# i2nico/MDAnalysis-MPI

Hardware: AMD Instinct MI355X
Metric: atom-frames/sec (RMSF) + achieved HBM GB/s fraction (higher is better)
Workload: dtype f64

## Files before the change

include/rmsf_hip.h:

```cpp
#ifndef RMSF_HIP_H
#define RMSF_HIP_H

#include <stddef.h>
#include <stdint.h>

#ifdef __cplusplus
extern "C" {
#endif

#define RMSF_ABI_VERSION 1

#define RMSF_OK 0
#define RMSF_EINVAL (-1)
#define RMSF_EHIP (-2)
#define RMSF_ENOMEM (-3)
#define RMSF_EEMPTY (-4)

#define RMSF_MODE_WELFORD 0
#define RMSF_MODE_SUM 1

#define RMSF_XFORM_DOUBLES 16
#define RMSF_MAX_SPLIT_FRAMES 4096
#define RMSF_REFINFO_DOUBLES 2064

// ... 15 lines not shown
int rmsf_reference_setup(const float *d_frame, const double *d_avg,
                         int64_t n_sel, const int32_t *d_sel,
                         const double *d_masses, double *d_ref,
                         double *d_refinfo, void *stream);

int rmsf_reference_setup_mean(const double *d_sum, double n_frames,
                              int64_t n_sel, const double *d_masses,
                              double *d_avg, double *d_ref, double *d_refinfo,
                              void *stream);

size_t rmsf_superpose_workspace_bytes(int64_t n_sel, int64_t n_frames);
int rmsf_superpose(const float *d_xyz, int64_t frame_stride, int64_t n_frames,
                   int64_t n_sel, const int32_t *d_sel,
                   const double *d_masses, const double *d_ref,
                   const double *d_refinfo, double *d_xform, void *d_work,
                   size_t work_bytes, void *stream);

int rmsf_superpose_compact(const float *d_xyz, int64_t frame_stride,
                           int64_t n_frames, int64_t n_sel, const int32_t *d_sel,
                           const double *d_masses, const double *d_ref,
                           const double *d_refinfo, double *d_xform,
                           void *d_work, size_t work_bytes, float *d_dense_out,
                           int64_t dense_stride, void *stream);

int rmsf_superpose_planes(const float *d_xyz, int64_t frame_stride,
                          int64_t plane_stride, int64_t n_frames,
                          int64_t n_sel, const int32_t *d_sel,
                          const double *d_masses, const double *d_ref,
                          const double *d_refinfo, double *d_xform,
                          void *d_work, size_t work_bytes, void *stream);

int rmsf_accumulate_splits(int64_t n_sel, int64_t n_frames, int aligned);
int rmsf_accumulate(const float *d_xyz, int64_t frame_stride, int64_t n_frames,
                    int64_t n_sel, const int32_t *d_sel,
                    const double *d_xform, const double *d_refinfo, int mode,
                    int n_splits, double *d_out0, double *d_out1,
                    void *stream);

int64_t rmsf_split_count(int64_t n_frames, int n_splits, int s);

size_t rmsf_accumulate_balanced_workspace_bytes(int64_t n_sel, int64_t n_frames,
                                                int n_groups);
int rmsf_accumulate_balanced(const float *d_xyz, int64_t frame_stride,
                             int64_t n_frames, int64_t n_sel,
                             const int32_t *d_sel, const double *d_xform,
                             const double *d_refinfo, int mode, int n_groups,
// ... 350 lines not shown
```

mdanalysis-mpi_amd/csrc/rmsf_device.h:

```cpp
#pragma once
#include <hip/hip_runtime.h>

#include <cmath>

__device__ __forceinline__ void apply_xform(float &x, float &y, float &z, const double *__restrict__ t,
                                            double rc0, double rc1, double rc2) {
  const float p0 = (float)((double)x - t[9]);
  const float p1 = (float)((double)y - t[10]);
  const float p2 = (float)((double)z - t[11]);
  const double d0 = p0, d1 = p1, d2 = p2;
  const float r0 = (float)__builtin_fma(d2, t[6], __builtin_fma(d1, t[3], d0 * t[0]));
  const float r1 = (float)__builtin_fma(d2, t[7], __builtin_fma(d1, t[4], d0 * t[1]));
  const float r2 = (float)__builtin_fma(d2, t[8], __builtin_fma(d1, t[5], d0 * t[2]));
  x = (float)((double)r0 + rc0);
  y = (float)((double)r1 + rc1);
  z = (float)((double)r2 + rc2);
}

__host__ __device__ inline void qcp_solve(const double *A, double E0, double len, double *rot,
                                          double *rmsd) {
  const double Sxx = A[0], Sxy = A[1], Sxz = A[2];
  const double Syx = A[3], Syy = A[4], Syz = A[5];
  const double Szx = A[6], Szy = A[7], Szz = A[8];

// ... 53 lines not shown
  const double evecprec = 1e-6;
  if (qsqr < evecprec) {
    q1 = a12 * a3344_4334 - a13 * a3244_4234 + a14 * a3243_4233;
    q2 = -a11 * a3344_4334 + a13 * a3144_4134 - a14 * a3143_4133;
    q3 = a11 * a3244_4234 - a12 * a3144_4134 + a14 * a3142_4132;
    q4 = -a11 * a3243_4233 + a12 * a3143_4133 - a13 * a3142_4132;
    qsqr = q1 * q1 + q2 * q2 + q3 * q3 + q4 * q4;
    if (qsqr < evecprec) {
      const double a1324_1423 = a13 * a24 - a14 * a23, a1224_1422 = a12 * a24 - a14 * a22;
      const double a1223_1322 = a12 * a23 - a13 * a22, a1124_1421 = a11 * a24 - a14 * a21;
      const double a1123_1321 = a11 * a23 - a13 * a21, a1122_1221 = a11 * a22 - a12 * a21;
      q1 = a42 * a1324_1423 - a43 * a1224_1422 + a44 * a1223_1322;
      q2 = -a41 * a1324_1423 + a43 * a1124_1421 - a44 * a1123_1321;
      q3 = a41 * a1224_1422 - a42 * a1124_1421 + a44 * a1122_1221;
      q4 = -a41 * a1223_1322 + a42 * a1123_1321 - a43 * a1122_1221;
      qsqr = q1 * q1 + q2 * q2 + q3 * q3 + q4 * q4;
      if (qsqr < evecprec) {
        q1 = a32 * a1324_1423 - a33 * a1224_1422 + a34 * a1223_1322;
        q2 = -a31 * a1324_1423 + a33 * a1124_1421 - a34 * a1123_1321;
        q3 = a31 * a1224_1422 - a32 * a1124_1421 + a34 * a1122_1221;
        q4 = -a31 * a1223_1322 + a32 * a1123_1321 - a33 * a1122_1221;
        qsqr = q1 * q1 + q2 * q2 + q3 * q3 + q4 * q4;
        if (qsqr < evecprec) {
          rot[0] = rot[4] = rot[8] = 1.0;
          rot[1] = rot[2] = rot[3] = rot[5] = rot[6] = rot[7] = 0.0;
          return;
        }
      }
    }
  }
  const double normq = sqrt(qsqr);
  q1 /= normq;
  q2 /= normq;
  q3 /= normq;
  q4 /= normq;
  const double a2 = q1 * q1, x2 = q2 * q2, y2 = q3 * q3, z2 = q4 * q4;
  const double xy = q2 * q3, az = q1 * q4, zx = q4 * q2, ay = q1 * q3, yz = q3 * q4, ax = q1 * q2;
  rot[0] = a2 + x2 - y2 - z2;
  rot[1] = 2 * (xy + az);
  rot[2] = 2 * (zx - ay);
  rot[3] = 2 * (xy - az);
  rot[4] = a2 - x2 + y2 - z2;
  rot[5] = 2 * (yz + ax);
  rot[6] = 2 * (zx + ay);
  rot[7] = 2 * (yz - ax);
  rot[8] = a2 - x2 - y2 + z2;
}
```

mdanalysis-mpi_amd/csrc/rmsf_kernels.hip:

```cpp
#include <hip/hip_runtime.h>

#include <algorithm>
#include <cmath>
#include <cstdint>
#include <cstring>
#include <mutex>
#include <string>
#include <type_traits>
#include <unordered_map>
#include <vector>

#include "rmsf_hip.h"
#include "rmsf_device.h"

#define RMSF_EXPORT __attribute__((visibility("default")))
#ifndef RMSF_SHIFTED_SUMS
#define RMSF_SHIFTED_SUMS 1
#endif

namespace {

thread_local std::string g_err;

int fail(int code, const std::string &msg) {
// ... 2814 lines not shown
    return fail(RMSF_EINVAL, "rmsf_welford_sequential: workspace too small");
  hipStream_t s = S(stream);
  SeqCoef *coef = static_cast<SeqCoef *>(d_work);
  hipLaunchKernelGGL(k_seq_coef, dim3(grid1(n_frames)), dim3(kBlock), 0, s, k0, n_frames, coef);
  if (int rc = after_launch("k_seq_coef")) return rc;
  const int64_t n_coord = 3 * n_sel;
  if (d_sel && n_sel >= kSeqAtomsMinSel) {
    hipLaunchKernelGGL((k_welford_seq_atoms<kSeqAtomsU>), dim3(grid1(n_sel)), dim3(kBlock), 0, s, d_xyz, fstride,
                       n_frames, n_sel, d_sel, k0, coef, d_mean, d_sumsquares);
    return after_launch("k_welford_seq_atoms");
  }
  if (d_sel)
    hipLaunchKernelGGL((k_welford_seq<kSeqU, true>), dim3(grid1(n_coord)), dim3(kBlock), 0, s, d_xyz, fstride,
                       n_frames, n_coord, d_sel, k0, coef, d_mean, d_sumsquares);
  else
    hipLaunchKernelGGL((k_welford_seq<kSeqU, false>), dim3(grid1(n_coord)), dim3(kBlock), 0, s, d_xyz, fstride,
                       n_frames, n_coord, nullptr, k0, coef, d_mean, d_sumsquares);
  return after_launch("k_welford_seq");
}

}

namespace {
bool ref_seq_args_ok(const float *d_frame, const double *d_avg, double avg_divisor, int64_t n_sel,
                     const int32_t *d_sel, const double *d_ref, const double *d_refinfo) {
  return (d_frame == nullptr) != (d_avg == nullptr) && n_sel >= 1 && d_ref && d_refinfo &&
         !(d_avg && !(avg_divisor > 0.0)) && !(d_avg && d_sel);
}
template <int PART>
void ref_seq_launch(const float *d_frame, const double *d_avg, double div, int64_t n_sel, const int32_t *d_sel,
                    const double *d_masses, double mass_total, double *d_avg_out, double *d_ref, double *d_refinfo,
                    hipStream_t s) {
  const bool g = d_sel != nullptr, m = d_masses != nullptr;
#define SEQREF(F, G, M)                                                                                          \
  hipLaunchKernelGGL((k_ref_seq<F, G, M, PART>), dim3(1), dim3(kBlock), 0, s, d_frame, d_avg, div, n_sel, d_sel, \
                     d_masses, mass_total, d_avg_out, d_ref, d_refinfo)
  if (d_frame) {
    if (g && m) SEQREF(true, true, true);
    else if (g) SEQREF(true, true, false);
    else if (m) SEQREF(true, false, true);
    else SEQREF(true, false, false);
  } else {
    if (m) SEQREF(false, false, true);
    else SEQREF(false, false, false);
  }
#undef SEQREF
// ... 303 lines not shown
```

mdanalysis-mpi_amd/rmsf_amd/_lib.py:

```python
from __future__ import annotations

import ctypes
import os
from ctypes import POINTER, c_char_p, c_double, c_int, c_int32, c_int64, c_size_t, c_uint64, c_void_p

_HERE = os.path.dirname(os.path.abspath(__file__))
LIB_PATH = os.path.normpath(os.path.join(_HERE, "..", "lib", "librmsf_hip.so"))

RMSF_OK = 0
RMSF_EINVAL = -1
RMSF_EHIP = -2
RMSF_ENOMEM = -3
RMSF_EEMPTY = -4
RMSF_MODE_WELFORD = 0
RMSF_MODE_SUM = 1
RMSF_XFORM_DOUBLES = 16
RMSF_MAX_SPLIT_FRAMES = 4096
RMSF_REFINFO_DOUBLES = 2064
ABI_VERSION = 1


class RmsfError(RuntimeError):

    def __init__(self, code: int, func: str, msg: str):
        super().__init__(f"{func} failed with status {code}: {msg}")
        self.code = code


class RmsfEmptyError(RmsfError, ZeroDivisionError):
    """No frames to reduce.  Subclasses ZeroDivisionError because RMSF.py:39
    raises exactly that when two empty partials are merged."""


P = c_void_p
SIGNATURES = {
    "rmsf_abi_version": (c_int, []),
    "rmsf_last_error": (c_char_p, []),
    "rmsf_device_count": (c_int, [POINTER(c_int)]),
    "rmsf_set_device": (c_int, [c_int]),
    "rmsf_malloc": (c_int, [POINTER(c_void_p), c_size_t]),
    "rmsf_free": (c_int, [P]),
    "rmsf_memcpy_h2d": (c_int, [P, P, c_size_t, P]),
    "rmsf_memcpy_d2h": (c_int, [P, P, c_size_t, P]),
    "rmsf_memcpy2d_d2d": (c_int, [P, c_size_t, P, c_size_t, c_size_t, c_size_t, P]),
    "rmsf_stream_synchronize": (c_int, [P]),
    "rmsf_block_range": (c_int, [c_int64, c_int, c_int, POINTER(c_int64), POINTER(c_int64)]),
    "rmsf_reference_setup": (c_int, [P, P, c_int64, P, P, P, P, P]),
    "rmsf_reference_setup_mean": (c_int, [P, c_double, c_int64, P, P, P, P, P]),
    "rmsf_fold_balanced_finalize": (c_int, [P, c_int64, c_int64, P, P, c_int64, P, P]),
    "rmsf_superpose_workspace_bytes": (c_size_t, [c_int64, c_int64]),
    "rmsf_superpose": (c_int, [P, c_int64, c_int64, c_int64, P, P, P, P, P, P, c_size_t, P]),
    "rmsf_superpose_planes": (c_int, [P, c_int64, c_int64, c_int64, c_int64, P, P, P, P, P, P, c_size_t, P]),
    "rmsf_superpose_compact": (c_int, [P, c_int64, c_int64, c_int64, P, P, P, P, P, P, c_size_t, P, c_int64, P]),
    "rmsf_accumulate_splits": (c_int, [c_int64, c_int64, c_int]),
    "rmsf_accumulate": (c_int, [P, c_int64, c_int64, c_int64, P, P, P, c_int, c_int, P, P, P]),
    "rmsf_split_count": (c_int64, [c_int64, c_int, c_int]),
    "rmsf_accumulate_balanced_workspace_bytes": (c_size_t, [c_int64, c_int64, c_int]),
    "rmsf_accumulate_balanced": (c_int, [P, c_int64, c_int64, c_int64, P, P, P, c_int, c_int, P, c_size_t, P]),
    "rmsf_fold_balanced": (c_int, [P, c_int64, c_int, c_int64, P, P, P]),
    "rmsf_accumulate_balanced_planes": (c_int, [P, c_int64, c_int64, c_int64, c_int64, P, P, P, c_int, c_int, P,
                                                c_size_t, P]),
    "rmsf_chan_merge": (c_int, [P, P, P, c_int, c_int64, P, P, P]),
    "rmsf_chan_reduce_steps": (c_int, [c_int, c_int, P, P, c_int]),
    "rmsf_chan_reduce": (c_int, [P, P, P, c_int, c_int64, c_int, P, P, P]),
    "rmsf_chan_merge_pair": (c_int, [P, P, c_int64, P, P, c_int64, c_int64, P]),
    "rmsf_sum_splits": (c_int, [P, c_int, c_int64, P, P]),
    "rmsf_divide": (c_int, [P, c_double, c_int64, P, P]),
    "rmsf_chan_weight": (c_int, [P, c_double, c_int64, P, P]),
    "rmsf_chan_deviation": (c_int, [P, P, P, c_double, c_int64, P, P]),
    "rmsf_finalize": (c_int, [P, c_int64, c_int64, P, P]),
    "rmsf_reference_setup_sequential": (c_int, [P, P, c_double, c_int64, P, P, c_double, P, P, P, P]),
    "rmsf_superpose_sequential": (c_int, [P, c_int64, c_int64, c_int64, P, P, c_double, P, P, P, P]),
    "rmsf_reference_centre_sequential": (c_int, [P, P, c_double, c_int64, P, P, c_double, P, P, P, P]),
    "rmsf_reference_sums_sequential": (c_int, [c_int64, c_double, P, P, P]),
    "rmsf_frame_com_sequential": (c_int, [P, c_int64, c_int64, c_int64, P, P, c_double, P, P]),
    "rmsf_inner_product_sequential": (c_int, [P, c_int64, c_int64, c_int64, P, P, P, P]),
# ... 171 lines not shown
```

mdanalysis-mpi_amd/rmsf_amd/engine.py:

```python
from __future__ import annotations

import ctypes

import numpy as np
import torch

from . import _lib
from ._lib import RMSF_MODE_SUM, RMSF_MODE_WELFORD, RMSF_REFINFO_DOUBLES, RMSF_XFORM_DOUBLES, call

F64 = torch.float64
F32 = torch.float32


def _ptr(t: torch.Tensor | None) -> int | None:
    return None if t is None else t.data_ptr()


class Engine:

    def __init__(self, device: torch.device | int | str | None = None):
        self.lib = _lib.load()
        if not torch.cuda.is_available():
            raise RuntimeError("rmsf_amd needs a HIP device (MI355X); none is visible -- no CPU fallback exists")
        if device is None:
# ... 40 lines not shown
        info = self.empty(RMSF_REFINFO_DOUBLES)
        call("rmsf_reference_setup_mean", total.data_ptr(), float(n_frames), n_sel, _ptr(masses), avg.data_ptr(),
             ref.data_ptr(), info.data_ptr(), self.stream)
        return avg, ref, info

    def workspace_bytes(self, n_sel: int, n_frames: int) -> int:
        return int(self.lib.rmsf_superpose_workspace_bytes(n_sel, n_frames))

    def superpose(self, xyz_ptr: int, fstride: int, n_frames: int, n_sel: int, sel, masses, ref, refinfo,
                  xform: torch.Tensor, work: torch.Tensor, pstride: int = 0, dense_out: int | None = None,
                  dense_stride: int = 0) -> None:
        if dense_out is not None:
            call("rmsf_superpose_compact", xyz_ptr, fstride, n_frames, n_sel, _ptr(sel), _ptr(masses),
                 ref.data_ptr(), refinfo.data_ptr(), xform.data_ptr(), work.data_ptr(),
                 work.numel() * work.element_size(), dense_out, dense_stride, self.stream)
            return
        if pstride:
            call("rmsf_superpose_planes", xyz_ptr, fstride, pstride, n_frames, n_sel, _ptr(sel), _ptr(masses),
                 ref.data_ptr(), refinfo.data_ptr(), xform.data_ptr(), work.data_ptr(),
                 work.numel() * work.element_size(), self.stream)
            return
        call("rmsf_superpose", xyz_ptr, fstride, n_frames, n_sel, _ptr(sel), _ptr(masses), ref.data_ptr(),
             refinfo.data_ptr(), xform.data_ptr(), work.data_ptr(), work.numel() * work.element_size(), self.stream)

    def splits(self, n_sel: int, n_frames: int, aligned: bool) -> int:
        return int(self.lib.rmsf_accumulate_splits(n_sel, n_frames, int(aligned)))

    def split_counts(self, n_frames: int, n_splits: int) -> list[int]:
        return [int(self.lib.rmsf_split_count(n_frames, n_splits, s)) for s in range(n_splits)]

    def accumulate(self, xyz_ptr: int, fstride: int, n_frames: int, n_sel: int, sel, xform, refinfo, mode: int,
                   n_splits: int, out0: torch.Tensor, out1: torch.Tensor | None) -> None:
        call("rmsf_accumulate", xyz_ptr, fstride, n_frames, n_sel, _ptr(sel), _ptr(xform), _ptr(refinfo), mode,
             n_splits, out0.data_ptr(), _ptr(out1), self.stream)

    def balanced_workspace_bytes(self, n_sel: int, n_frames: int, n_groups: int = 0) -> int:
        return int(self.lib.rmsf_accumulate_balanced_workspace_bytes(n_sel, n_frames, n_groups))

    def accumulate_balanced(self, xyz_ptr: int, fstride: int, n_frames: int, n_sel: int, sel, xform, refinfo,
                            mode: int, work: torch.Tensor, n_groups: int = 0, pstride: int = 0) -> None:
        if pstride:
            call("rmsf_accumulate_balanced_planes", xyz_ptr, fstride, pstride, n_frames, n_sel, _ptr(sel),
                 _ptr(xform), _ptr(refinfo), mode, n_groups, work.data_ptr(), work.numel() * work.element_size(),
                 self.stream)
            return
        call("rmsf_accumulate_balanced", xyz_ptr, fstride, n_frames, n_sel, _ptr(sel), _ptr(xform), _ptr(refinfo),
# ... 256 lines not shown
```

mdanalysis-mpi_amd/rmsf_amd/pipeline.py:

```python
from __future__ import annotations

import contextlib
import os
from collections import defaultdict
from dataclasses import dataclass, field

import numpy as np
import torch

from . import parallel
from ._lib import (RMSF_MAX_SPLIT_FRAMES, RMSF_MODE_SUM, RMSF_MODE_WELFORD, RMSF_REFINFO_DOUBLES, RMSF_XFORM_DOUBLES,
                   RmsfEmptyError)
from .engine import Engine
from .sources import Batch, DeviceSource, FrameList, _scattered

ALIGN_MODES = (None, "frame0", "average")


class KernelTimer:

    def __init__(self):
        self.spans = defaultdict(list)

    @contextlib.contextmanager
    def span(self, name: str, atom_frames: int = 0):
        s = torch.cuda.current_stream()
        a = torch.cuda.Event(enable_timing=True)
        b = torch.cuda.Event(enable_timing=True)
        a.record(s)
        yield
        b.record(s)
        self.spans[name].append((a, b, int(atom_frames)))

    def clear(self) -> None:
        self.spans.clear()

    def ms(self, name: str) -> list[float]:
        torch.cuda.synchronize()
        return [a.elapsed_time(b) for a, b, _ in self.spans.get(name, [])]

    def totals(self, name: str) -> tuple[int, float, int]:
        t = self.ms(name)
        return len(t), float(sum(t)), sum(af for _, _, af in self.spans.get(name, []))


_NULL = contextlib.nullcontext()


def _span(timer, name, atom_frames: int = 0):
    return timer.span(name, atom_frames) if timer is not None else _NULL


class Accumulator:

    def __init__(self, eng: Engine, n_sel: int, mode: int, max_batch: int, aligned: bool,
                 n_splits: int | None = None, timer: KernelTimer | None = None):
        self.eng, self.n_sel, self.mode, self.aligned = eng, n_sel, mode, aligned
        self.timer = timer
        self.n_coord = 3 * n_sel
        self.fixed_splits = n_splits
        self.work = None
        if n_splits:
            self.s_max = max(n_splits, -(-max_batch // RMSF_MAX_SPLIT_FRAMES))
        else:
            self.s_max = 0
            nbytes = eng.balanced_workspace_bytes(n_sel, max_batch)
            self.work = eng.empty(max(2, (nbytes + 7) // 8))
        self.parts0 = eng.empty(1 + self.s_max, self.n_coord)
        self.parts1 = None
        if mode == RMSF_MODE_WELFORD:
            self.parts1 = eng.empty(1 + self.s_max, self.n_coord)
        self.n = 0
        self.packed = False
# ... 31 lines not shown
                else:
                    eng.fold_balanced_shift(self.work, self.n_coord, self.n, self.parts0[0], p1, shift, off3, t)
                self.packed = True
            elif fin is not None and self.mode == RMSF_MODE_WELFORD and self.aligned:
                eng.fold_balanced_finalize(self.work, self.n_coord, self.n, self.parts0[0], p1, fin[1], fin[0])
                self.finalized = True
            else:
                eng.fold_balanced(self.work, self.n_coord, self.mode, self.n, self.parts0[0], p1)
            self.n += b.n_frames
            return
        if b.pstride:
            raise ValueError("coordinate planes are read in place on the balanced grid only (n_splits=None)")
        s = max(self.fixed_splits, -(-b.n_frames // RMSF_MAX_SPLIT_FRAMES))
        with _span(self.timer, "accumulate", b.n_frames * self.n_sel):
            eng.accumulate(b.ptr, b.fstride, b.n_frames, self.n_sel, b.sel, xform, refinfo, self.mode, s,
                           self.parts0[1:], None if self.parts1 is None else self.parts1[1:])
        if self.mode == RMSF_MODE_WELFORD:
            counts = [self.n] + eng.split_counts(b.n_frames, s)
            eng.chan_merge(self.parts0, self.parts1, counts, self.n_coord, self.parts0[0], self.parts1[0])
        else:
            eng.sum_splits(self.parts0, 1 + s, self.n_coord, self.parts0[0])
        self.n += b.n_frames

    @property
    def result0(self) -> torch.Tensor:
        if self.n == 0:
            self._zero()
        return self.parts0[0]

    @property
    def result1(self) -> torch.Tensor:
        if self.n == 0:
            self._zero()
        return self.parts1[0]


class CovarianceAccumulator:

    def __init__(self, eng: Engine, n_sel: int, max_batch: int, shift: torch.Tensor,
                 timer: KernelTimer | None = None):
        self.eng, self.n_sel, self.timer = eng, n_sel, timer
        self.n_coord = n = 3 * n_sel
        check_covariance_memory(eng, n_sel)
        if shift.dtype != torch.float64 or shift.numel() != n:
            raise ValueError("the covariance shift is f64 [3 n_sel]")
        self.shift = shift.reshape(-1)
# ... 70 lines not shown
    if shift_work is not None:
        shift_work.wait()
    return shift.double()


class Superposer:

    def __init__(self, eng: Engine, n_sel: int, max_batch: int, masses: torch.Tensor | None,
                 timer: KernelTimer | None = None):
        self.eng, self.n_sel, self.masses, self.timer = eng, n_sel, masses, timer
        self.xform = eng.empty(max_batch, RMSF_XFORM_DOUBLES)
        nbytes = eng.workspace_bytes(n_sel, max_batch)
        self.work = eng.empty(max(1, (nbytes + 7) // 8))

    def run(self, b: Batch, ref: torch.Tensor, refinfo: torch.Tensor, dense_out: int | None = None,
            dense_stride: int = 0) -> torch.Tensor:
        xf = self.xform[: b.n_frames]
        need = self.eng.workspace_bytes(self.n_sel, b.n_frames)
        if need > self.work.numel() * 8:
            self.work = self.eng.empty((need + 7) // 8)
        with _span(self.timer, "superpose", b.n_frames * self.n_sel):
            self.eng.superpose(b.ptr, b.fstride, b.n_frames, self.n_sel, b.sel, self.masses, ref, refinfo, xf,
                               self.work, pstride=b.pstride, dense_out=dense_out, dense_stride=dense_stride)
        return xf


COMPACT_MAX_DENSITY = 0.5
COMPACT_MAX_DENSITY_ONE_SWEEP = 0.2


class _Compactor:

    max_bytes: int | None = None

    def __init__(self, eng: Engine, n_sel: int, n_local: int, max_batch: int):
        self.n_sel = n_sel
        self.pitch = (3 * n_sel + 3) // 4 * 4
        row = 4 * self.pitch
        budget = self.max_bytes
        if budget is None:
            budget = torch.cuda.mem_get_info(eng.device)[0] // 2
        cap = max(1, budget // row)
        self.resident = n_local <= cap
        self.frames = n_local if self.resident else max(1, min(max_batch, cap))
        self.usable = self.resident or self.frames >= max_batch
        self.buf = None
# ... 203 lines not shown
            raise ValueError("masses must have one entry per selected atom")
    aligned = align is not None
    planes = not aligned and not n_splits and bool(getattr(source, "native_planes", False))
    if scatter and planes:
        raise ValueError("merge_scatter: the statistics of coordinate planes read in place are in plane order, "
                         "not atom order; use merge_root")
    batches_of = source.raw_batches if planes else source.batches
    if not planes and not n_splits and isinstance(source, DeviceSource) and source.layout == "soa":
        batches_of = source.plane_batches_in_place
    gathered = (aligned and not planes and isinstance(source, DeviceSource) and source.layout == "fac"
                and source.sel_dev is not None and not _scattered_block(frames, b0, b1, max_batch))
    if compact is None:
        dmax = COMPACT_MAX_DENSITY if align == "average" else COMPACT_MAX_DENSITY_ONE_SWEEP
        compact = gathered and n_sel <= dmax * source.n_atoms
    cmp = _Compactor(eng, n_sel, n_local, max_batch) if (compact and gathered and n_local) else None
    if cmp is not None and not cmp.usable:
        cmp = None
    sup = Superposer(eng, n_sel, max_batch, m_dev, timer) if aligned else None
    rmsd = eng.empty(n_local) if (aligned and collect_rmsd) else None
    keep = aligned and collect_transforms
    xf_last = eng.empty(n_local, RMSF_XFORM_DOUBLES) if keep else None
    xf_first = eng.empty(n_local, RMSF_XFORM_DOUBLES) if (keep and align == "average") else None
    average = None

    def sweep(acc: Accumulator, ref=None, info=None, xf_out=None, pack=None, slabs=None, fin=None, cov=None):
        done, slabbed = 0, None
        if cmp is not None and cmp.resident and cmp.filled:
            batches = cmp.resident_batches(n_local, max_batch)
        else:
            batches = batches_of(frames, b0, b1, max_batch, eng.stream)
        for b in batches:
            xf, src_b = None, b
            if aligned:
                if cmp is not None and b.sel is not None:
                    k = done if cmp.resident else 0
                    xf = sup.run(b, ref, info, dense_out=cmp.ptr(k), dense_stride=cmp.pitch)
                    b = cmp.dense(k, b.n_frames)
                else:
                    xf = sup.run(b, ref, info)
                if rmsd is not None:
                    rmsd[done:done + b.n_frames].copy_(xf[:, 12])
                if xf_out is not None:
                    xf_out[done:done + b.n_frames].copy_(xf)
            last = done + b.n_frames == n_local
            if slabs and done == 0 and last and b.sel is None and xf is None and not b.pstride:
                n_chunks = eng.balanced_slab_chunks(b.ptr, b.fstride, b.n_frames, n_sel)
                if n_chunks >= 2 * 3:
                    shift_, off3_, _, work_ = pack[:4]
                    slabbed = _slab_sweep(eng, acc, b, _slab_bounds(n_chunks, slabs), shift_, off3_, work_, timer,
                                          root)
            if slabbed is None:
                acc.add(b, xf, info, pack if last else None, fin if last else None)
            if cov is not None:
                cov.add(b, xf, info)
            done += b.n_frames
            src_b.done()
        if cmp is not None and cmp.resident:
            cmp.filled = True
        return slabbed

    if align == "average":
        ref0, info0 = reference_from_frame(eng, source, ref_frame, n_sel, m_dev, ref_owner)
        acc1 = Accumulator(eng, n_sel, RMSF_MODE_SUM, max_batch, True, n_splits, timer)
        if n_local:
            sweep(acc1, ref0, info0, xf_first)
        total = parallel.allreduce_sum_(acc1.result0)
        average, ref, info = eng.reference_setup_mean(total, float(n_total), n_sel, m_dev)
    elif align == "frame0":
        ref, info = reference_from_frame(eng, source, ref_frame, n_sel, m_dev, ref_owner)
    else:
        ref = info = None

    shift = off3 = shift_work = None
    if size > 1:
# ... 10 lines not shown
         if size > 1 else None)
    k_slabs = merge_slabs if merge_slabs is not None else (SLABS_AUTO if n_sel >= SLAB_MIN_ATOMS else 0)
    slabs = k_slabs if (size > 1 and k_slabs > 1 and not aligned and not n_splits and not scatter
                        and not covariance) else None
    slabbed = None
    rmsf_fin = eng.empty(n_sel) if (size == 1 and aligned) else None
    covacc = comoment = None
    if covariance:
        covacc = CovarianceAccumulator(eng, n_sel, max_batch,
                                       _covariance_shift(eng, source, frames, align, average, ref, info, shift,
                                                         shift_work), timer)
    if n_local:
        slabbed = sweep(acc, ref, info, xf_last, (shift, off3, t, shift_work, sc) if size > 1 else None, slabs,
                        (rmsf_fin, n_total) if rmsf_fin is not None else None, covacc)
    if covacc is not None:
        comoment = covacc.finish(n_total, root)
    if slabbed is not None:
        if root is not None and rank != root:
            with _span(timer, "merge"):
                for *_, work in slabbed:
                    if work is not None:
                        work.wait()
            return PipelineResult(rmsf=None, mean=None, m2=None, n_frames=n_total, n_local=n_local, block=(b0, b1),
                                  average=None, rmsd=rmsd, extras={"merge_slabs": len(slabbed), "merge_root": root})
        mean, m2, rmsf = eng.empty(3 * n_sel), eng.empty(3 * n_sel), eng.empty(n_sel)
        with _span(timer, "merge"):
            for t_k, j0, j1, work in slabbed:
                if work is not None:
                    work.wait()
                eng.chan_shift_finish(t_k, shift[j0:j1], off3, (j1 - j0) // 3, n_total, mean[j0:j1], m2[j0:j1],
                                      rmsf[j0 // 3:j1 // 3])
        if planes:
            mean, m2, rmsf = _rows_from_planes(eng, mean, m2, n_sel, n_total)
        return PipelineResult(rmsf=rmsf, mean=mean.view(n_sel, 3), m2=m2.view(n_sel, 3), n_frames=n_total,
                              n_local=n_local, block=(b0, b1), average=None, rmsd=rmsd,
                              extras={"merge_slabs": len(slabbed), "merge_root": root})
    if scatter:
        with _span(timer, "merge"):
            rmsf, mean_s, m2_s, (a0, a1) = parallel.global_chan_scatter(
                eng, acc.result0, acc.result1, acc.n, n_total, shift, off3, None if acc.packed else shift_work,
                packed=t if acc.packed else None, slice_coords=sc, root=root)
        return PipelineResult(rmsf=rmsf, mean=None, m2=None, n_frames=n_total, n_local=n_local, block=(b0, b1),
                              average=None if average is None else average.view(n_sel, 3), rmsd=rmsd,
                              transforms=xf_last, transforms_sweep1=xf_first,
                              extras={"merge_root": root, "merge": "scatter", "atom_slice": (a0, a1),
                                      "slice_mean": mean_s.view(-1, 3), "slice_m2": m2_s.view(-1, 3)})
    if size > 1:
        with _span(timer, "merge"):
            mean, m2, rmsf = parallel.global_chan_shifted(eng, acc.result0, acc.result1, acc.n, n_total,
                                                          shift, off3, None if acc.packed else shift_work,
                                                          packed=t if acc.packed else None, root=root)
        if planes and rmsf is not None:
            mean, m2, rmsf = _rows_from_planes(eng, mean, m2, n_sel, n_total)
        if rmsf is None:
            return PipelineResult(rmsf=None, mean=None, m2=None, n_frames=n_total, n_local=n_local,
                                  block=(b0, b1), average=None if average is None else average.view(n_sel, 3),
                                  rmsd=rmsd, transforms=xf_last, transforms_sweep1=xf_first,
                                  extras={"merge_root": root}, comoment=comoment)
    elif planes:
        mean, m2, rmsf = _rows_from_planes(eng, acc.result0, acc.result1, n_sel, n_total)
    else:
        mean, m2 = acc.result0, acc.result1
        if acc.finalized:
            rmsf = rmsf_fin
        else:
            rmsf = eng.empty(n_sel)
            eng.finalize(m2, n_sel, n_total, rmsf)
    return PipelineResult(rmsf=rmsf, mean=mean.view(n_sel, 3), m2=m2.view(n_sel, 3), n_frames=n_total,
                          n_local=n_local, block=(b0, b1),
                          average=None if average is None else average.view(n_sel, 3), rmsd=rmsd,
                          transforms=xf_last, transforms_sweep1=xf_first, comoment=comoment)


EXACT_OVERLAP_MIN_ATOMS = 16384


def _run_exact(eng: Engine, source, frames: FrameList, max_batch, block, timer, merge_root,
               merge_order: str = "mpi4py", *, align=None, masses=None, ref_frame: int = 0,
               ref_owner: int | None = None, collect_rmsd: bool = False,
               collect_transforms: bool = False, covariance: bool = False) -> PipelineResult:
    rank, size = parallel.world()
    n_total = len(frames)
    if n_total == 0:
        raise RmsfEmptyError(-4, "RMSF.run", "no frames selected")
    if merge_root is not None and not 0 <= merge_root < size:
        raise ValueError(f"merge_root {merge_root} is not a rank of this {size}-rank group")
    root = merge_root if size > 1 else None
    blocks = parallel.blocks(n_total, size)
    if block is not None and size > 1 and tuple(block) != blocks[rank]:
        raise ValueError(f"rank {rank}: block {tuple(block)} is not the RMSF.py:65-69 block {blocks[rank]}")
    b0, b1 = block if block is not None else blocks[rank]
    n_local = b1 - b0
    n_sel = source.n_sel
    max_batch = max(1, min(max_batch or max(1, n_local), max(1, n_local)))
# ... 119 lines not shown

class UploadedMasses:

    def __init__(self, masses, device):
        self.host = np.ascontiguousarray(masses, dtype=np.float64)
        self.dev = torch.as_tensor(self.host).to(device)

    def __len__(self) -> int:
        return self.host.size


class CapturedPipeline:

    def __init__(self, eng: Engine, source, frames: FrameList, **kw):
        from .sources import DeviceSource

        if parallel.world()[1] > 1:
            raise NotImplementedError("graph capture is single-process (the RCCL merge is not captured)")
        if not isinstance(source, DeviceSource):
            raise TypeError("only HBM-resident (DeviceSource) pipelines can be captured")
        if kw.get("timer") is not None:
            raise ValueError("a KernelTimer cannot be captured")
        dev = eng.device
        if kw.get("masses") is not None and not isinstance(kw["masses"], UploadedMasses):
            kw["masses"] = UploadedMasses(kw["masses"], dev)
        side = torch.cuda.Stream(dev)
        side.wait_stream(torch.cuda.current_stream(dev))
        with torch.cuda.stream(side):
            run_pipeline(eng, source, frames, **kw)
        torch.cuda.current_stream(dev).wait_stream(side)
        self.graph = torch.cuda.CUDAGraph()
        with torch.cuda.graph(self.graph):
            self.result = run_pipeline(eng, source, frames, **kw)

    def replay(self) -> PipelineResult:
        self.graph.replay()
        return self.result
```

Before: 548.7 billion.

## Add fused single-pass superpose+accumulate kernel for small selections

Adds a k_small_sweep kernel for selections of up to 512 atoms. Each wave owns a contiguous frame range, computes the QCP superposition, applies the transform and accumulates per-atom moments in registers or LDS, all in one read of the coordinates instead of separate superpose and accumulate passes. A k_small_finish kernel reduces the per-block partials, merges them into the running accumulator and can finalize RMSF. The pipeline takes this path automatically when the selection is small and there are enough frames, which saves a second pass over HBM and several launches, at the cost of one wave doing a full serial QCP solve per frame.

```diff
diff --git a/include/rmsf_hip.h b/include/rmsf_hip.h
--- a/include/rmsf_hip.h
+++ b/include/rmsf_hip.h
@@ -61,6 +61,21 @@
                            const double *d_refinfo, double *d_xform,
                            void *d_work, size_t work_bytes, float *d_dense_out,
                            int64_t dense_stride, void *stream);
+
+#define RMSF_SMALL_SEL 512
+int rmsf_small_sweep_plan(int64_t n_frames, int n_cu, int *n_groups,
+                          int *n_waves);
+int rmsf_small_sweep_range(int64_t n_frames, int n_waves, int w, int64_t *lo,
+                           int64_t *hi);
+size_t rmsf_small_sweep_workspace_bytes(int64_t n_sel, int64_t n_frames);
+int rmsf_small_sweep(const float *d_xyz, int64_t frame_stride,
+                     int64_t plane_stride, int64_t n_frames, int64_t n_sel,
+                     const int32_t *d_sel, const double *d_masses,
+                     const double *d_ref, const double *d_refinfo, int mode,
+                     double *d_xform, float *d_dense_out, int64_t dense_stride,
+                     void *d_work, size_t work_bytes, int64_t acc_n,
+                     double *d_acc0, double *d_acc1, int64_t n_total,
+                     double *d_rmsf, void *stream);
 
 int rmsf_superpose_planes(const float *d_xyz, int64_t frame_stride,
                           int64_t plane_stride, int64_t n_frames,
diff --git a/mdanalysis-mpi_amd/csrc/rmsf_device.h b/mdanalysis-mpi_amd/csrc/rmsf_device.h
--- a/mdanalysis-mpi_amd/csrc/rmsf_device.h
+++ b/mdanalysis-mpi_amd/csrc/rmsf_device.h
@@ -99,9 +99,8 @@
         q4 = -a31 * a1223_1322 + a32 * a1123_1321 - a33 * a1122_1221;
         qsqr = q1 * q1 + q2 * q2 + q3 * q3 + q4 * q4;
         if (qsqr < evecprec) {
-          rot[0] = rot[4] = rot[8] = 1.0;
-          rot[1] = rot[2] = rot[3] = rot[5] = rot[6] = rot[7] = 0.0;
-          return;
+          q1 = qsqr = 1.0;
+          q2 = q3 = q4 = 0.0;
         }
       }
     }
diff --git a/mdanalysis-mpi_amd/csrc/rmsf_kernels.hip b/mdanalysis-mpi_amd/csrc/rmsf_kernels.hip
--- a/mdanalysis-mpi_amd/csrc/rmsf_kernels.hip
+++ b/mdanalysis-mpi_amd/csrc/rmsf_kernels.hip
@@ -2860,6 +2860,356 @@
 }
 
 namespace {
+
+constexpr int kSmallSel = RMSF_SMALL_SEL;
+constexpr int kSmallWaves = 8;
+constexpr int kSmallThreads = 64 * kSmallWaves;
+static_assert(kSmallSel == 64 * 8, "k_small_sweep: at most 8 atoms per lane");
+
+__host__ __device__ inline int64_t small_lo(int64_t n_frames, int n_waves, int w) {
+  return n_frames * w / n_waves;
+}
+
+int small_groups(int64_t n_frames, int n_cu) {
+  if (n_cu <= 0) n_cu = cu_count();
+  const int64_t g = (n_frames + kSmallWaves - 1) / kSmallWaves;
+  return (int)std::max<int64_t>(1, std::min<int64_t>(g, n_cu));
+}
+
+template <int APL, int MODE, bool GATHER, bool MASSES>
+__global__ __launch_bounds__(kSmallThreads) void k_small_sweep(
+    const float *__restrict__ xyz, int64_t fstride, int64_t n_frames, int n_sel, const int32_t *__restrict__ sel,
+    const double *__restrict__ masses, const double *__restrict__ ref, const double *__restrict__ refinfo,
+    double *__restrict__ xform, float *__restrict__ dense, int64_t dpitch, double *__restrict__ part) {
+  constexpr int NV = MODE == RMSF_MODE_WELFORD ? 2 : 1;
+  constexpr int NC = 3 * 64 * APL;
+  __shared__ double s_ref[NC];
+  __shared__ double s_mass[MASSES ? 64 * APL : 1];
+  constexpr bool QL = APL == 8 && MODE == RMSF_MODE_WELFORD;
+  __shared__ double s_sum[(QL ? 1 : NV) * NC];
+  __shared__ double s_q[QL ? kSmallWaves * NC : 1];
+  const int lane = threadIdx.x & 63;
+  const int w = __builtin_amdgcn_readfirstlane(threadIdx.x >> 6);
+  const int n3 = 3 * n_sel;
+  for (int j = threadIdx.x; j < NC; j += kSmallThreads) s_ref[j] = j < n3 ? ref[j] : 0.0;
+  if (MASSES)
+    for (int j = threadIdx.x; j < 64 * APL; j += kSmallThreads) s_mass[j] = j < n_sel ? masses[j] : 0.0;
+  __syncthreads();
+
+  const int n_waves = (int)gridDim.x * kSmallWaves;
+  const int gw = (int)blockIdx.x * kSmallWaves + w;
+  const int64_t f_lo = uni64(small_lo(n_frames, n_waves, gw));
+  const int64_t f_hi = uni64(small_lo(n_frames, n_waves, gw + 1));
+  const double rc0 = refinfo[0], rc1 = refinfo[1], rc2 = refinfo[2];
+  const double sr0 = refinfo[3], sr1 = refinfo[4], sr2 = refinfo[5];
+  const double gref = refinfo[6], mtot = refinfo[7], nsel = refinfo[8];
+
+  int32_t at[APL];
+#pragma unroll
+  for (int k = 0; k < APL; ++k) {
+    const int a = min(lane + 64 * k, n_sel - 1);
+    at[k] = GATHER ? sel[a] : a;
+  }
+  double m[APL][3], q[APL][3];
+#pragma unroll
+  for (int k = 0; k < APL; ++k)
+#pragma unroll
+    for (int c = 0; c < 3; ++c) {
+      m[k][c] = q[k][c] = 0.0;
+      if (QL) s_q[w * NC + 3 * (lane + 64 * k) + c] = 0.0;
+    }
+
+  float cur[3 * APL], nxt[3 * APL];
+  auto load = [&](float(&v)[3 * APL], int64_t f) {
+    const float *fr = xyz + f * fstride;
+#pragma unroll
+    for (int k = 0; k < APL; ++k) {
+      const float *p = fr + 3 * (int64_t)at[k];
+      v[3 * k] = __builtin_nontemporal_load(p);
+      v[3 * k + 1] = __builtin_nontemporal_load(p + 1);
+      v[3 * k + 2] = __builtin_nontemporal_load(p + 2);
+    }
+  };
+  if (f_lo < f_hi) load(cur, f_lo);
+  for (int64_t f = f_lo; f < f_hi; ++f) {
+    load(nxt, min(f + 1, f_hi - 1));
+    if (dense) {
+      float *drow = dense + f * dpitch;
+#pragma unroll
+      for (int k = 0; k < APL; ++k) {
+        const int a = lane + 64 * k;
+        if (a < n_sel) {
+          drow[3 * a] = cur[3 * k];
+          drow[3 * a + 1] = cur[3 * k + 1];
+          drow[3 * a + 2] = cur[3 * k + 2];
+        }
+      }
+    }
+    const double px = (double)__shfl(cur[0], 0, 64), py = (double)__shfl(cur[1], 0, 64),
+                 pz = (double)__shfl(cur[2], 0, 64);
+    double acc[kStats];
+#pragma unroll
+    for (int j = 0; j < kStats; ++j) acc[j] = 0.0;
+#pragma unroll
+    for (int k = 0; k < APL; ++k) {
+      const int a = lane + 64 * k;
+      if (a < n_sel) {
+        const double r0 = s_ref[3 * a], r1 = s_ref[3 * a + 1], r2 = s_ref[3 * a + 2];
+        const double x = (double)cur[3 * k] - px, y = (double)cur[3 * k + 1] - py, z = (double)cur[3 * k + 2] - pz;
+        acc[0] += x;
+        acc[1] += y;
+        acc[2] += z;
+        if (MASSES) {
+          const double ms = s_mass[a];
+          acc[3] = fma(ms, x, acc[3]);
+          acc[4] = fma(ms, y, acc[4]);
+          acc[5] = fma(ms, z, acc[5]);
+        }
+        acc[6] = fma(x, r0, acc[6]);
+        acc[7] = fma(x, r1, acc[7]);
+        acc[8] = fma(x, r2, acc[8]);
+        acc[9] = fma(y, r0, acc[9]);
+        acc[10] = fma(y, r1, acc[10]);
+        acc[11] = fma(y, r2, acc[11]);
+        acc[12] = fma(z, r0, acc[12]);
+        acc[13] = fma(z, r1, acc[13]);
+        acc[14] = fma(z, r2, acc[14]);
+        acc[15] = fma(x, x, fma(y, y, fma(z, z, acc[15])));
+      }
+    }
+    wave_sum(acc);
+    const double cx = (MASSES ? acc[3] : acc[0]) / mtot;
+    const double cy = (MASSES ? acc[4] : acc[1]) / mtot;
+    const double cz = (MASSES ? acc[5] : acc[2]) / mtot;
+    double A[9];
+    A[0] = acc[6] - cx * sr0;
+    A[1] = acc[7] - cx * sr1;
+    A[2] = acc[8] - cx * sr2;
+    A[3] = acc[9] - cy * sr0;
+    A[4] = acc[10] - cy * sr1;
+    A[5] = acc[11] - cy * sr2;
+    A[6] = acc[12] - cz * sr0;
+    A[7] = acc[13] - cz * sr1;
+    A[8] = acc[14] - cz * sr2;
+    const double gmob =
+        acc[15] - 2.0 * (cx * acc[0] + cy * acc[1] + cz * acc[2]) + nsel * (cx * cx + cy * cy + cz * cz);
+    const double E0 = 0.5 * (gmob + gref);
+    double t[12], rmsd;
+    qcp_solve(A, E0, nsel, t, &rmsd);
+    t[9] = px + cx;
+    t[10] = py + cy;
+    t[11] = pz + cz;
+    if (lane == 0) {
+      double *o = xform + f * kXform;
+#pragma unroll
+      for (int j = 0; j < 12; ++j) o[j] = t[j];
+      o[12] = rmsd;
+      o[13] = o[14] = o[15] = 0.0;
+    }
+#pragma unroll
+    for (int k = 0; k < APL; ++k) {
+      const int a = lane + 64 * k;
+      if (a < n_sel) {
+        float x = cur[3 * k], y = cur[3 * k + 1], z = cur[3 * k + 2];
+        apply_xform(x, y, z, t, rc0, rc1, rc2);
+        if (MODE == RMSF_MODE_WELFORD) {
+          const double d0 = (double)x - (s_ref[3 * a] + rc0), d1 = (double)y - (s_ref[3 * a + 1] + rc1),
+                       d2 = (double)z - (s_ref[3 * a + 2] + rc2);
+          m[k][0] += d0, m[k][1] += d1, m[k][2] += d2;
+          if (QL) {
+            double *sq = s_q + w * NC + 3 * a;
+            sq[0] = fma(d0, d0, sq[0]), sq[1] = fma(d1, d1, sq[1]), sq[2] = fma(d2, d2, sq[2]);
+          } else {
+            q[k][0] = fma(d0, d0, q[k][0]), q[k][1] = fma(d1, d1, q[k][1]), q[k][2] = fma(d2, d2, q[k][2]);
+          }
+        } else {
+          m[k][0] += (double)x, m[k][1] += (double)y, m[k][2] += (double)z;
+        }
+      }
+    }
+#pragma unroll
+    for (int j = 0; j < 3 * APL; ++j) cur[j] = nxt[j];
+  }
+
+  for (int v = 0; v < kSmallWaves; ++v) {
+    if (w == v) {
+#pragma unroll
+      for (int k = 0; k < APL; ++k) {
+#pragma unroll
+        for (int c = 0; c < 3; ++c) {
+          const int j = 3 * (lane + 64 * k) + c;
+          s_sum[j] = v == 0 ? m[k][c] : s_sum[j] + m[k][c];
+          if (NV == 2 && !QL) s_sum[NC + j] = v == 0 ? q[k][c] : s_sum[NC + j] + q[k][c];
+        }
+      }
+    }
+    __syncthreads();
+  }
+  double *out = part + (int64_t)blockIdx.x * NV * n3;
+  for (int j = threadIdx.x; j < n3; j += kSmallThreads) {
+    out[j] = s_sum[j];
+    if (QL) {
+      double t2 = s_q[j];
+#pragma unroll
+      for (int v = 1; v < kSmallWaves; ++v) t2 += s_q[v * NC + j];
+      out[n3 + j] = t2;
+    } else if (NV == 2) {
+      out[n3 + j] = s_sum[NC + j];
+    }
+  }
+}
+
+constexpr int kFinCoords = 24, kFinSlices = 10, kFinU = 8;
+static_assert(kFinCoords % 3 == 0 && kFinCoords * kFinSlices <= kBlock, "k_small_finish: block shape");
+
+__global__ __launch_bounds__(kBlock) void k_small_finish(const double *__restrict__ part, int groups, int n3,
+                                                         int mode, double nf, const double *__restrict__ ref,
+                                                         const double *__restrict__ refinfo, double acc_n,
+                                                         double *__restrict__ acc0, double *__restrict__ acc1,
+                                                         double n_total, double *__restrict__ rmsf) {
+  __shared__ double red[2][kFinSlices][kFinCoords];
+  const bool wel = mode == RMSF_MODE_WELFORD;
+  const int nv = wel ? 2 : 1;
+  const int c = threadIdx.x % kFinCoords, s = threadIdx.x / kFinCoords;
+  const int j = (int)blockIdx.x * kFinCoords + c;
+  if (s < kFinSlices) {
+    double s1 = 0.0, s2 = 0.0;
+    if (j < n3) {
+      const int g1 = groups * (s + 1) / kFinSlices;
+      int g = groups * s / kFinSlices;
+      const double *p = part + j;
+      const int64_t gs = (int64_t)nv * n3;
+      for (; g + kFinU <= g1; g += kFinU) {
+        double v1[kFinU], v2[kFinU];
+#pragma unroll
+        for (int u = 0; u < kFinU; ++u) {
+          v1[u] = p[(g + u) * gs];
+          v2[u] = wel ? p[(g + u) * gs + n3] : 0.0;
+        }
+#pragma unroll
+        for (int u = 0; u < kFinU; ++u) s1 += v1[u], s2 += v2[u];
+      }
+      for (; g < g1; ++g) {
+        s1 += p[g * gs];
+        if (wel) s2 += p[g * gs + n3];
+      }
+    }
+    red[0][s][c] = s1;
+    red[1][s][c] = s2;
+  }
+  __syncthreads();
+  if (s == 0 && j < n3) {
+    double s1 = red[0][0][c], s2 = red[1][0][c];
+#pragma unroll
+    for (int v = 1; v < kFinSlices; ++v) s1 += red[0][v][c], s2 += red[1][v][c];
+    if (!wel) {
+      acc0[j] = acc_n > 0 ? acc0[j] + s1 : s1;
+    } else {
+      shifted_to_moments(s1, s2, ref[j] + refinfo[j % 3], 1.0 / nf);
+      double mu = s1, M = s2;
+      if (acc_n > 0) {
+        const double n1 = acc_n, n2 = nf, mu1 = acc0[j], M1 = acc1[j];
+        const double T = n1 + n2;
+        const double d = mu - mu1;
+        mu = (n1 * mu1 + n2 * mu) / T;
+        M = M1 + M + (n1 * n2 / T) * (d * d);
+      }
+      acc0[j] = mu;
+      acc1[j] = M;
+      red[1][0][c] = M;
+    }
+  }
+  __syncthreads();
+  if (wel && rmsf && threadIdx.x < kFinCoords / 3) {
+    const int a = (int)blockIdx.x * (kFinCoords / 3) + threadIdx.x;
+    if (3 * a + 2 < n3)
+      rmsf[a] = sqrt((red[1][0][3 * threadIdx.x] + red[1][0][3 * threadIdx.x + 1] + red[1][0][3 * threadIdx.x + 2]) /
+                     n_total);
+  }
+}
+
+}
+
+extern "C" {
+
+RMSF_EXPORT int rmsf_small_sweep_plan(int64_t n_frames, int n_cu, int *n_groups, int *n_waves) {
+  if (n_frames < 0 || !n_groups || !n_waves) return fail(RMSF_EINVAL, "rmsf_small_sweep_plan: bad arguments");
+  *n_groups = small_groups(n_frames, n_cu);
+  *n_waves = *n_groups * kSmallWaves;
+  return RMSF_OK;
+}
+
+RMSF_EXPORT int rmsf_small_sweep_range(int64_t n_frames, int n_waves, int w, int64_t *lo, int64_t *hi) {
+  if (n_frames < 0 || n_waves < 1 || w < 0 || w >= n_waves || !lo || !hi)
+    return fail(RMSF_EINVAL, "rmsf_small_sweep_range: bad arguments");
+  *lo = small_lo(n_frames, n_waves, w);
+  *hi = small_lo(n_frames, n_waves, w + 1);
+  return RMSF_OK;
+}
+
+RMSF_EXPORT size_t rmsf_small_sweep_workspace_bytes(int64_t n_sel, int64_t n_frames) {
+  if (n_sel < 1 || n_sel > kSmallSel || n_frames < 0) return 0;
+  return (size_t)small_groups(n_frames, 0) * 2 * 3 * (size_t)n_sel * sizeof(double);
+}
+
+RMSF_EXPORT int rmsf_small_sweep(const float *d_xyz, int64_t fstride, int64_t plane_stride, int64_t n_frames,
+                                 int64_t n_sel, const int32_t *d_sel, const double *d_masses, const double *d_ref,
+                                 const double *d_refinfo, int mode, double *d_xform, float *d_dense_out,
+                                 int64_t dense_stride, void *d_work, size_t work_bytes, int64_t acc_n,
+                                 double *d_acc0, double *d_acc1, int64_t n_total, double *d_rmsf, void *stream) {
+  if (plane_stride != 0)
+    return fail(RMSF_EINVAL, "rmsf_small_sweep: coordinate planes take the two-pass path (rmsf_superpose_planes)");
+  if (n_sel > kSmallSel)
+    return fail(RMSF_EINVAL, "rmsf_small_sweep: n_sel > RMSF_SMALL_SEL takes the two-pass path (rmsf_superpose)");
+  if (mode != RMSF_MODE_WELFORD && mode != RMSF_MODE_SUM) return fail(RMSF_EINVAL, "rmsf_small_sweep: bad mode");
+  if (n_frames == 0) return RMSF_OK;
+  if (!d_xyz || !d_ref || !d_refinfo || !d_xform || !d_work || !d_acc0 || (mode == RMSF_MODE_WELFORD && !d_acc1) ||
+      n_sel < 1 || n_frames < 0 || acc_n < 0 || fstride < (d_sel ? 3 : 3 * n_sel) ||
+      (d_rmsf && (mode != RMSF_MODE_WELFORD || n_total < 1)))
+    return fail(RMSF_EINVAL, "rmsf_small_sweep: bad arguments");
+  if (d_dense_out) {
+    if (!d_sel) return fail(RMSF_EINVAL, "rmsf_small_sweep: the dense copy is of a gathered selection");
+    if (dense_stride == 0) dense_stride = 3 * n_sel;
+    if (dense_stride < 3 * n_sel) return fail(RMSF_EINVAL, "rmsf_small_sweep: dense_stride < 3 n_sel");
+  }
+  if (work_bytes < rmsf_small_sweep_workspace_bytes(n_sel, n_frames))
+    return fail(RMSF_ENOMEM, "rmsf_small_sweep: workspace too small");
+  hipStream_t s = S(stream);
+  const int groups = small_groups(n_frames, 0);
+  double *part = static_cast<double *>(d_work);
+  const bool g = d_sel != nullptr, ms = d_masses != nullptr;
+#define SMALL_LAUNCH(APL_, M_, G_, W_)                                                                             \
+  hipLaunchKernelGGL((k_small_sweep<APL_, M_, G_, W_>), dim3(groups), dim3(kSmallThreads), 0, s, d_xyz, fstride,  \
+                     n_frames, (int)n_sel, d_sel, d_masses, d_ref, d_refinfo, d_xform, d_dense_out, dense_stride, \
+                     part)
+#define SMALL_GW(APL_, M_)                     \
+  do {                                         \
+    if (g && ms) SMALL_LAUNCH(APL_, M_, true, true);        \
+    else if (g) SMALL_LAUNCH(APL_, M_, true, false);        \
+    else if (ms) SMALL_LAUNCH(APL_, M_, false, true);       \
+    else SMALL_LAUNCH(APL_, M_, false, false);              \
+  } while (0)
+  if (n_sel <= 256) {
+    if (mode == RMSF_MODE_WELFORD) SMALL_GW(4, RMSF_MODE_WELFORD);
+    else SMALL_GW(4, RMSF_MODE_SUM);
+  } else {
+    if (mode == RMSF_MODE_WELFORD) SMALL_GW(8, RMSF_MODE_WELFORD);
+    else SMALL_GW(8, RMSF_MODE_SUM);
+  }
+#undef SMALL_GW
+#undef SMALL_LAUNCH
+  int rc = after_launch("k_small_sweep");
+  if (rc) return rc;
+  const int n3 = 3 * (int)n_sel;
+  hipLaunchKernelGGL(k_small_finish, dim3((n3 + kFinCoords - 1) / kFinCoords), dim3(kBlock), 0, s, part, groups, n3,
+                     mode, (double)n_frames, d_ref, d_refinfo, (double)acc_n, d_acc0, d_acc1, (double)n_total,
+                     d_rmsf);
+  return after_launch("k_small_finish");
+}
+
+}
+
+namespace {
 bool ref_seq_args_ok(const float *d_frame, const double *d_avg, double avg_divisor, int64_t n_sel,
                      const int32_t *d_sel, const double *d_ref, const double *d_refinfo) {
   return (d_frame == nullptr) != (d_avg == nullptr) && n_sel >= 1 && d_ref && d_refinfo &&
diff --git a/mdanalysis-mpi_amd/rmsf_amd/_lib.py b/mdanalysis-mpi_amd/rmsf_amd/_lib.py
--- a/mdanalysis-mpi_amd/rmsf_amd/_lib.py
+++ b/mdanalysis-mpi_amd/rmsf_amd/_lib.py
@@ -17,6 +17,7 @@
 RMSF_XFORM_DOUBLES = 16
 RMSF_MAX_SPLIT_FRAMES = 4096
 RMSF_REFINFO_DOUBLES = 2064
+RMSF_SMALL_SEL = 512
 ABI_VERSION = 1
 
 
@@ -52,6 +53,11 @@
     "rmsf_superpose": (c_int, [P, c_int64, c_int64, c_int64, P, P, P, P, P, P, c_size_t, P]),
     "rmsf_superpose_planes": (c_int, [P, c_int64, c_int64, c_int64, c_int64, P, P, P, P, P, P, c_size_t, P]),
     "rmsf_superpose_compact": (c_int, [P, c_int64, c_int64, c_int64, P, P, P, P, P, P, c_size_t, P, c_int64, P]),
+    "rmsf_small_sweep_plan": (c_int, [c_int64, c_int, POINTER(c_int), POINTER(c_int)]),
+    "rmsf_small_sweep_range": (c_int, [c_int64, c_int, c_int, POINTER(c_int64), POINTER(c_int64)]),
+    "rmsf_small_sweep_workspace_bytes": (c_size_t, [c_int64, c_int64]),
+    "rmsf_small_sweep": (c_int, [P, c_int64, c_int64, c_int64, c_int64, P, P, P, P, c_int, P, P, c_int64, P, c_size_t,
+                                 c_int64, P, P, c_int64, P, P]),
     "rmsf_accumulate_splits": (c_int, [c_int64, c_int64, c_int]),
     "rmsf_accumulate": (c_int, [P, c_int64, c_int64, c_int64, P, P, P, c_int, c_int, P, P, P]),
     "rmsf_split_count": (c_int64, [c_int64, c_int, c_int]),
diff --git a/mdanalysis-mpi_amd/rmsf_amd/engine.py b/mdanalysis-mpi_amd/rmsf_amd/engine.py
--- a/mdanalysis-mpi_amd/rmsf_amd/engine.py
+++ b/mdanalysis-mpi_amd/rmsf_amd/engine.py
@@ -86,6 +86,19 @@
             return
         call("rmsf_superpose", xyz_ptr, fstride, n_frames, n_sel, _ptr(sel), _ptr(masses), ref.data_ptr(),
              refinfo.data_ptr(), xform.data_ptr(), work.data_ptr(), work.numel() * work.element_size(), self.stream)
+
+    def small_sweep_workspace_bytes(self, n_sel: int, n_frames: int) -> int:
+        return int(self.lib.rmsf_small_sweep_workspace_bytes(n_sel, n_frames))
+
+    def small_sweep(self, xyz_ptr: int, fstride: int, n_frames: int, n_sel: int, sel, masses, ref, refinfo,
+                    mode: int, xform: torch.Tensor, work: torch.Tensor, acc_n: int, acc0: torch.Tensor,
+                    acc1: torch.Tensor | None, dense_out: int | None = None, dense_stride: int = 0,
+                    fin=None, pstride: int = 0) -> None:
+        rmsf, n_total = fin if fin is not None else (None, 0)
+        call("rmsf_small_sweep", xyz_ptr, fstride, pstride, n_frames, n_sel, _ptr(sel), _ptr(masses),
+             ref.data_ptr(), refinfo.data_ptr(), mode, xform.data_ptr(), dense_out, dense_stride, work.data_ptr(),
+             work.numel() * work.element_size(), acc_n, acc0.data_ptr(), _ptr(acc1), n_total, _ptr(rmsf),
+             self.stream)
 
     def splits(self, n_sel: int, n_frames: int, aligned: bool) -> int:
         return int(self.lib.rmsf_accumulate_splits(n_sel, n_frames, int(aligned)))
diff --git a/mdanalysis-mpi_amd/rmsf_amd/pipeline.py b/mdanalysis-mpi_amd/rmsf_amd/pipeline.py
--- a/mdanalysis-mpi_amd/rmsf_amd/pipeline.py
+++ b/mdanalysis-mpi_amd/rmsf_amd/pipeline.py
@@ -9,8 +9,8 @@
 import torch
 
 from . import parallel
-from ._lib import (RMSF_MAX_SPLIT_FRAMES, RMSF_MODE_SUM, RMSF_MODE_WELFORD, RMSF_REFINFO_DOUBLES, RMSF_XFORM_DOUBLES,
-                   RmsfEmptyError)
+from ._lib import (RMSF_MAX_SPLIT_FRAMES, RMSF_MODE_SUM, RMSF_MODE_WELFORD, RMSF_REFINFO_DOUBLES, RMSF_SMALL_SEL,
+                   RMSF_XFORM_DOUBLES, RmsfEmptyError)
 from .engine import Engine
 from .sources import Batch, DeviceSource, FrameList, _scattered
 
@@ -49,6 +49,23 @@
 
 def _span(timer, name, atom_frames: int = 0):
     return timer.span(name, atom_frames) if timer is not None else _NULL
+
+
+SMALL_SWEEP_MIN_FRAMES = 1024
+
+
+def small_sweep_forced() -> bool | None:
+    v = os.environ.get("RMSF_SMALL_SWEEP")
+    return None if v in (None, "") else bool(int(v))
+
+
+def use_small_sweep(n_sel: int, n_frames: int, *, pstride: int = 0, n_splits=None, merge_scatter: bool = False,
+                    merge_slabs=None, forced: bool | None = None) -> bool:
+    if forced is False or n_frames < 1:
+        return False
+    if n_sel > RMSF_SMALL_SEL or pstride or n_splits or merge_scatter or merge_slabs not in (None, 0, 1):
+        return False
+    return bool(forced) or n_frames >= SMALL_SWEEP_MIN_FRAMES
 
 
 class Accumulator:
@@ -126,6 +143,17 @@
             eng.sum_splits(self.parts0, 1 + s, self.n_coord, self.parts0[0])
         self.n += b.n_frames
 
+    def add_small(self, b: Batch, sup: "Superposer", ref: torch.Tensor, refinfo: torch.Tensor,
+                  dense_out: int | None = None, dense_stride: int = 0, fin=None) -> torch.Tensor:
+        if self.mode != RMSF_MODE_WELFORD:
+            fin = None
+        xf = sup.small_sweep(b, ref, refinfo, self.mode, self.n, self.parts0[0],
+                             None if self.parts1 is None else self.parts1[0], dense_out, dense_stride, fin)
+        self.n += b.n_frames
+        if fin is not None:
+            self.finalized = True
+        return xf
+
     @property
     def result0(self) -> torch.Tensor:
         if self.n == 0:
@@ -242,6 +270,20 @@
         with _span(self.timer, "superpose", b.n_frames * self.n_sel):
             self.eng.superpose(b.ptr, b.fstride, b.n_frames, self.n_sel, b.sel, self.masses, ref, refinfo, xf,
                                self.work, pstride=b.pstride, dense_out=dense_out, dense_stride=dense_stride)
+        return xf
+
+    def small_sweep(self, b: Batch, ref: torch.Tensor, refinfo: torch.Tensor, mode: int, acc_n: int,
+                    acc0: torch.Tensor, acc1: torch.Tensor | None, dense_out: int | None = None,
+                    dense_stride: int = 0, fin=None) -> torch.Tensor:
+        xf = self.xform[: b.n_frames]
+        need = self.eng.small_sweep_workspace_bytes(self.n_sel, b.n_frames)
+        work = getattr(self, "small_work", None)
+        if work is None or need > work.numel() * 8:
+            work = self.small_work = self.eng.empty(max(1, (need + 7) // 8))
+        with _span(self.timer, "superpose", b.n_frames * self.n_sel):
+            self.eng.small_sweep(b.ptr, b.fstride, b.n_frames, self.n_sel, b.sel, self.masses, ref, refinfo, mode, xf,
+                                 work, acc_n, acc0, acc1, dense_out=dense_out, dense_stride=dense_stride, fin=fin,
+                                 pstride=b.pstride)
         return xf
 
 
@@ -491,6 +533,8 @@
     xf_last = eng.empty(n_local, RMSF_XFORM_DOUBLES) if keep else None
     xf_first = eng.empty(n_local, RMSF_XFORM_DOUBLES) if (keep and align == "average") else None
     average = None
+    forced = small_sweep_forced()
+    paths = {"small_sweep_batches": 0, "two_pass_batches": 0}
 
     def sweep(acc: Accumulator, ref=None, info=None, xf_out=None, pack=None, slabs=None, fin=None, cov=None):
         done, slabbed = 0, None
@@ -500,7 +544,24 @@
             batches = batches_of(frames, b0, b1, max_batch, eng.stream)
         for b in batches:
             xf, src_b = None, b
+            last = done + b.n_frames == n_local
+            fused = aligned and use_small_sweep(n_sel, b.n_frames, pstride=b.pstride, n_splits=n_splits,
+                                                merge_scatter=merge_scatter, merge_slabs=merge_slabs, forced=forced)
             if aligned:
+                paths["small_sweep_batches" if fused else "two_pass_batches"] += 1
+            if fused:
+                if cmp is not None and b.sel is not None and ((align == "average" and cmp.resident)
+                                                              or cov is not None):
+                    k = done if cmp.resident else 0
+                    xf = acc.add_small(b, sup, ref, info, cmp.ptr(k), cmp.pitch, fin if last else None)
+                    b = cmp.dense(k, b.n_frames)
+                else:
+                    xf = acc.add_small(b, sup, ref, info, fin=fin if last else None)
+                if rmsd is not None:
+                    rmsd[done:done + b.n_frames].copy_(xf[:, 12])
+                if xf_out is not None:
+                    xf_out[done:done + b.n_frames].copy_(xf)
+            elif aligned:
                 if cmp is not None and b.sel is not None:
                     k = done if cmp.resident else 0
                     xf = sup.run(b, ref, info, dense_out=cmp.ptr(k), dense_stride=cmp.pitch)
@@ -511,14 +572,13 @@
                     rmsd[done:done + b.n_frames].copy_(xf[:, 12])
                 if xf_out is not None:
                     xf_out[done:done + b.n_frames].copy_(xf)
-            last = done + b.n_frames == n_local
             if slabs and done == 0 and last and b.sel is None and xf is None and not b.pstride:
                 n_chunks = eng.balanced_slab_chunks(b.ptr, b.fstride, b.n_frames, n_sel)
                 if n_chunks >= 2 * 3:
                     shift_, off3_, _, work_ = pack[:4]
                     slabbed = _slab_sweep(eng, acc, b, _slab_bounds(n_chunks, slabs), shift_, off3_, work_, timer,
                                           root)
-            if slabbed is None:
+            if slabbed is None and not fused:
                 acc.add(b, xf, info, pack if last else None, fin if last else None)
             if cov is not None:
                 cov.add(b, xf, info)
@@ -575,7 +635,7 @@
                     if work is not None:
                         work.wait()
             return PipelineResult(rmsf=None, mean=None, m2=None, n_frames=n_total, n_local=n_local, block=(b0, b1),
-                                  average=None, rmsd=rmsd, extras={"merge_slabs": len(slabbed), "merge_root": root})
+                                  average=None, rmsd=rmsd, extras={"merge_slabs": len(slabbed), "merge_root": root, **paths})
         mean, m2, rmsf = eng.empty(3 * n_sel), eng.empty(3 * n_sel), eng.empty(n_sel)
         with _span(timer, "merge"):
             for t_k, j0, j1, work in slabbed:
@@ -587,7 +647,7 @@
             mean, m2, rmsf = _rows_from_planes(eng, mean, m2, n_sel, n_total)
         return PipelineResult(rmsf=rmsf, mean=mean.view(n_sel, 3), m2=m2.view(n_sel, 3), n_frames=n_total,
                               n_local=n_local, block=(b0, b1), average=None, rmsd=rmsd,
-                              extras={"merge_slabs": len(slabbed), "merge_root": root})
+                              extras={"merge_slabs": len(slabbed), "merge_root": root, **paths})
     if scatter:
         with _span(timer, "merge"):
             rmsf, mean_s, m2_s, (a0, a1) = parallel.global_chan_scatter(
@@ -597,7 +657,7 @@
                               average=None if average is None else average.view(n_sel, 3), rmsd=rmsd,
                               transforms=xf_last, transforms_sweep1=xf_first,
                               extras={"merge_root": root, "merge": "scatter", "atom_slice": (a0, a1),
-                                      "slice_mean": mean_s.view(-1, 3), "slice_m2": m2_s.view(-1, 3)})
+                                      "slice_mean": mean_s.view(-1, 3), "slice_m2": m2_s.view(-1, 3), **paths})
     if size > 1:
         with _span(timer, "merge"):
             mean, m2, rmsf = parallel.global_chan_shifted(eng, acc.result0, acc.result1, acc.n, n_total,
@@ -609,7 +669,7 @@
             return PipelineResult(rmsf=None, mean=None, m2=None, n_frames=n_total, n_local=n_local,
                                   block=(b0, b1), average=None if average is None else average.view(n_sel, 3),
                                   rmsd=rmsd, transforms=xf_last, transforms_sweep1=xf_first,
-                                  extras={"merge_root": root}, comoment=comoment)
+                                  extras={"merge_root": root, **paths}, comoment=comoment)
     elif planes:
         mean, m2, rmsf = _rows_from_planes(eng, acc.result0, acc.result1, n_sel, n_total)
     else:
@@ -622,7 +682,7 @@
     return PipelineResult(rmsf=rmsf, mean=mean.view(n_sel, 3), m2=m2.view(n_sel, 3), n_frames=n_total,
                           n_local=n_local, block=(b0, b1),
                           average=None if average is None else average.view(n_sel, 3), rmsd=rmsd,
-                          transforms=xf_last, transforms_sweep1=xf_first, comoment=comoment)
+                          transforms=xf_last, transforms_sweep1=xf_first, extras=dict(paths), comoment=comoment)
 
 
 EXACT_OVERLAP_MIN_ATOMS = 16384
@@ -788,6 +848,7 @@
         if kw.get("timer") is not None:
             raise ValueError("a KernelTimer cannot be captured")
         dev = eng.device
+        self.source = source
         if kw.get("masses") is not None and not isinstance(kw["masses"], UploadedMasses):
             kw["masses"] = UploadedMasses(kw["masses"], dev)
         side = torch.cuda.Stream(dev)
```

Result: slower. 543.0 billion (-1.0%).
